# piotrmwojcik/GI-GS

Hardware: AMD Instinct MI355X
Metric: train-step renders/sec (fwd+bwd, G-buffer+indirect) at 800x800; PSNR vs the CPU oracle (higher is better)
Workload: dtype f32; 1 GPU; C2 (configs[1] TensoIR lego stand-in): 300k surface Gaussians, 800x800, SH deg 2, GI step=16 start=8 delta=0.0625; P=300000, N=640000, M=9, hip_graphs=on, fused_glue=on, gi_march=proj, rasterizer=whole step = 2 hand-captured hipGraphs (fwd, bwd), asynchronous binning

## Files before the change

gi-gs_amd/csrc/pbr.hip:

```cpp
#include <cmath>
#include <cstdlib>
#include <cstring>
#include <map>
#include <mutex>
#include <vector>

#include "gigs_common.h"
#include "pixel_ops.h"

namespace gigs {

__device__ __forceinline__ v3 safe_normalize(v3 v) {
  const float l = sqrtf(v.x * v.x + v.y * v.y + v.z * v.z);
  return l > 0.0f ? v3{v.x / l, v.y / l, v.z / l} : v3{0, 0, 0};
}
__device__ __forceinline__ v3 cube_dir_raw(float fx, float fy, int side) {
  switch (side) {
    case 0: return {1, -fy, -fx};
    case 1: return {-1, -fy, fx};
    case 2: return {fx, 1, fy};
    case 3: return {fx, -1, -fy};
    case 4: return {fx, -fy, 1};
    default: return {-fx, -fy, -1};
  }
}
__device__ __forceinline__ v3 cube_to_dir(int x, int y, int side, int N) {
  const float fx = 2.0f * (((float)x + 0.5f) / (float)N) - 1.0f;
  const float fy = 2.0f * (((float)y + 0.5f) / (float)N) - 1.0f;
  return safe_normalize(cube_dir_raw(fx, fy, side));
}
__device__ __forceinline__ float ndf_ggx(float alphaSqr, float cosTheta) {
  const float c = fminf(fmaxf(cosTheta, 0.0f), 1.0f);
  const float d = (c * alphaSqr - c) * c + 1.0f;
  return (float)((double)alphaSqr / ((double)(d * d) * 3.14159265358979323846));
}

__global__ void __launch_bounds__(256)
texel_table_kernel(int N, const float* __restrict__ area, float4* __restrict__ table) {
  const int o = blockIdx.x * 256 + threadIdx.x;
  if (o >= 6 * N * N) return;
  const int pz = o / (N * N), py = (o / N) % N, px = o % N;
  const v3 d = cube_to_dir(px, py, pz, N);
  float a = 1.0f;
  if (N > 1) {
    const int Hh = N / 2;
    a = area[abs(px - Hh)] * area[abs(py - Hh)];
  }
  table[o] = make_float4(d.x, d.y, d.z, a);
}

struct TexelTable { float4* dev = nullptr; };
static std::mutex g_table_mu;
static std::map<long long, TexelTable> g_table;

static const float4* texel_table(int N, hipStream_t s) {
  int dev = 0;
  if (hipGetDevice(&dev) != hipSuccess) return nullptr;
  std::lock_guard<std::mutex> lk(g_table_mu);
  const long long key = ((long long)dev << 32) | (unsigned)N;
  auto it = g_table.find(key);
  if (it != g_table.end()) return it->second.dev;
  const int Hh = N / 2;
  std::vector<float> h(Hh + 2, 1.0f);
  if (N > 1)
    for (int i = 0; i <= Hh; i++) h[i] = atanf((float)(i + 1) / (float)Hh) - atanf((float)i / (float)Hh);
  float* area = nullptr;
  TexelTable t;
  if (hipMalloc(&area, h.size() * sizeof(float)) != hipSuccess) return nullptr;
  if (hipMalloc(&t.dev, (size_t)6 * N * N * sizeof(float4)) != hipSuccess) return nullptr;
  if (hipMemcpyAsync(area, h.data(), h.size() * sizeof(float), hipMemcpyHostToDevice, s) != hipSuccess) return nullptr;
  hipLaunchKernelGGL(texel_table_kernel, dim3((6 * N * N + 255) / 256), dim3(256), 0, s, N, area, t.dev);
  if (hipStreamSynchronize(s) != hipSuccess) return nullptr;
  hipFree(area);
  g_table[key] = t;
  return t.dev;
}

template <int kCtrl, int kRowMask = 0xf>
__device__ __forceinline__ float pbr_dpp(float v) {
  return __int_as_float(__builtin_amdgcn_update_dpp(0, __float_as_int(v), kCtrl, kRowMask, 0xf, false));
}
__device__ __forceinline__ float wave_sum63(float v) {
  v += pbr_dpp<0xb1>(v);
  v += pbr_dpp<0x4e>(v);
  v += pbr_dpp<0x124>(v);
  v += pbr_dpp<0x128>(v);
  v += pbr_dpp<0x142, 0xa>(v);
  v += pbr_dpp<0x143, 0xc>(v);
  return v;
}

template <bool kBackward>
__global__ void __launch_bounds__(256)
diffuse_cubemap_kernel(int N, const float4* __restrict__ table, const float* __restrict__ src,
                       float* __restrict__ dst) {
  const int o = blockIdx.x * 4 + (threadIdx.x >> 6);
  const int lane = threadIdx.x & 63;
  if (o >= 6 * N * N) return;
  const float4 me = table[o];
  float c0 = 0, c1 = 0, c2 = 0;
  for (int i = lane; i < 6 * N * N; i += 64) {
    const float4 ot = table[i];
    const float d = kBackward ? (ot.x * me.x + ot.y * me.y + ot.z * me.z) : (me.x * ot.x + me.y * ot.y + me.z * ot.z);
    const float costheta = fminf(fmaxf(d, 0.0f), 0.999f);
    const float w = costheta * (kBackward ? me.w : ot.w) / 3.141592f;
    const float* t = src + 3 * (size_t)i;
    c0 += t[0] * w; c1 += t[1] * w; c2 += t[2] * w;
  }
  c0 = wave_sum63(c0); c1 = wave_sum63(c1); c2 = wave_sum63(c2);
  if (lane == 63) { dst[3 * (size_t)o] = c0; dst[3 * (size_t)o + 1] = c1; dst[3 * (size_t)o + 2] = c2; }
}


__global__ void __launch_bounds__(64)
specular_bounds_kernel(int N, float cutoff, float* __restrict__ bounds) {
  const int o = blockIdx.x * 64 + threadIdx.x;
  if (o >= 6 * N * N) return;
  const int pz = o / (N * N), py = (o / N) % N, px = o % N;
  const v3 VNR = cube_to_dir(px, py, pz, N);
  const int TILE = 16;
  for (int s = 0; s < 6; ++s) {
    int minx = N - 1, maxx = 0, miny = N - 1, maxy = 0;
    for (int tx = 0; tx < (N + TILE - 1) / TILE; tx++)
      for (int ty = 0; ty < (N + TILE - 1) / TILE; ty++) {
        const int tsx = tx * TILE, tsy = ty * TILE;
        const int tex = min((tx + 1) * TILE, N), tey = min((ty + 1) * TILE, N);
        const v3 L0 = cube_to_dir(tsx, tsy, s, N), L1 = cube_to_dir(tex, tsy, s, N);
        const v3 L2 = cube_to_dir(tsx, tey, s, N), L3 = cube_to_dir(tex, tey, s, N);
        const float mnx = fminf(fminf(L0.x, L1.x), fminf(L2.x, L3.x)), mxx = fmaxf(fmaxf(L0.x, L1.x), fmaxf(L2.x, L3.x));
        const float mny = fminf(fminf(L0.y, L1.y), fminf(L2.y, L3.y)), mxy = fmaxf(fmaxf(L0.y, L1.y), fmaxf(L2.y, L3.y));
        const float mnz = fminf(fminf(L0.z, L1.z), fminf(L2.z, L3.z)), mxz = fmaxf(fmaxf(L0.z, L1.z), fmaxf(L2.z, L3.z));
        const float maxdp = fmaxf(mnx * VNR.x, mxx * VNR.x) + fmaxf(mny * VNR.y, mxy * VNR.y) + fmaxf(mnz * VNR.z, mxz * VNR.z);
        if (maxdp >= cutoff) {
          for (int y = tsy; y < tey; ++y)
            for (int x = tsx; x < tex; ++x) {
              const v3 L = cube_to_dir(x, y, s, N);
              if (dot3(L, VNR) >= cutoff) {
                minx = min(minx, x); maxx = max(maxx, x);
                miny = min(miny, y); maxy = max(maxy, y);
              }
            }
        }
      }
    float* b = bounds + 24 * (size_t)o + s * 4;
    b[0] = (float)minx; b[1] = (float)maxx; b[2] = (float)miny; b[3] = (float)maxy;
  }
}

__device__ __forceinline__ v3 normalize_exact(v3 v) {
  const float l = sqrtf(v.x * v.x + v.y * v.y + v.z * v.z);
  if (!(l > 0x1p-60f && l < 0x1p60f)) return safe_normalize(v);
  const float r0 = __builtin_amdgcn_rcpf(l);
  const float e0 = __builtin_fmaf(-l, r0, 1.0f);
  const float r1 = __builtin_fmaf(e0, r0, r0);
  v3 q;
  {
    const float q0 = v.x * r1, e1 = __builtin_fmaf(-l, q0, v.x), q1 = __builtin_fmaf(e1, r1, q0);
    q.x = __builtin_fmaf(__builtin_fmaf(-l, q1, v.x), r1, q1);
  }
  {
    const float q0 = v.y * r1, e1 = __builtin_fmaf(-l, q0, v.y), q1 = __builtin_fmaf(e1, r1, q0);
    q.y = __builtin_fmaf(__builtin_fmaf(-l, q1, v.y), r1, q1);
  }
  {
    const float q0 = v.z * r1, e1 = __builtin_fmaf(-l, q0, v.z), q1 = __builtin_fmaf(e1, r1, q0);
    q.z = __builtin_fmaf(__builtin_fmaf(-l, q1, v.z), r1, q1);
  }
  return q;
}

template <bool kBackward>
__global__ void __launch_bounds__(256)
specular_cubemap_kernel(int N, const float4* __restrict__ table, const float* __restrict__ src,
                        const float* __restrict__ bounds, float roughness, float cutoff,
                        float* __restrict__ dst) {
  const int o = blockIdx.x * 4 + (threadIdx.x >> 6);
  const int lane = threadIdx.x & 63;
  if (o >= 6 * N * N) return;
  const int lx = lane & 7, ly = lane >> 3;
  const float4 me = table[o];
  const float alpha = roughness * roughness, alphaSqr = alpha * alpha;
  float wsum = 0.0f, c0 = 0, c1 = 0, c2 = 0;
  const int stride = kBackward ? 4 : 3;
  const float4* b4 = reinterpret_cast<const float4*>(bounds + 24 * (size_t)o);
  for (int s = 0; s < 6; ++s) {
    const float4 b = b4[s];
    const int xmin = (int)b.x, xmax = (int)b.y, ymin = (int)b.z, ymax = (int)b.w;
    if (xmin > xmax) continue;
    for (int y = ymin + ly; y <= ymax; y += 8)
      for (int x = xmin + lx; x <= xmax; x += 8) {
        const int i = (s * N + y) * N + x;
        const float4 ot = table[i];
        const float d = kBackward ? (me.x * ot.x + me.y * ot.y + me.z * ot.z) : (ot.x * me.x + ot.y * me.y + ot.z * me.z);
        if (d >= cutoff) {
          const float wiDotN = fmaxf(d, 0.0f);
          const v3 Hh = kBackward ? normalize_exact(v3{me.x + ot.x, me.y + ot.y, me.z + ot.z})
                                  : normalize_exact(v3{ot.x + me.x, ot.y + me.y, ot.z + me.z});
          const float VNRDotH = fmaxf(kBackward ? (ot.x * Hh.x + ot.y * Hh.y + ot.z * Hh.z)
                                                : (me.x * Hh.x + me.y * Hh.y + me.z * Hh.z), 0.0f);
          const float c = fminf(fmaxf(VNRDotH, 0.0f), 1.0f);
          const float dd = (c * alphaSqr - c) * c + 1.0f;
          const float ndf = alphaSqr / ((dd * dd) * 3.14159265358979323846f);
          const float w = wiDotN * ndf * (kBackward ? me.w : ot.w) / 4.0f;
          const float* t = src + (size_t)stride * i;
          c0 += t[0] * w; c1 += t[1] * w; c2 += t[2] * w;
          wsum += w;
        }
      }
  }
  c0 = wave_sum63(c0); c1 = wave_sum63(c1); c2 = wave_sum63(c2);
  if (!kBackward) wsum = wave_sum63(wsum);
  if (lane == 63) {
    if (kBackward) {
      float* q = dst + 3 * (size_t)o;
      q[0] = c0; q[1] = c1; q[2] = c2;
    } else {
      float* q = dst + 4 * (size_t)o;
      q[0] = c0; q[1] = c1; q[2] = c2; q[3] = wsum;
    }
  }
}


template <bool kSwap>
__global__ void __launch_bounds__(256)
specular_weights_kernel(int N, const float4* __restrict__ table, const float* __restrict__ bounds,
                        const uint32_t* __restrict__ offsets, float roughness, float cutoff,
                        float* __restrict__ W) {
  const int o = blockIdx.x * 4 + (threadIdx.x >> 6);
  const int lane = threadIdx.x & 63;
  if (o >= 6 * N * N) return;
  const float4 me = table[o];
  const float alpha = roughness * roughness, alphaSqr = alpha * alpha;
  const float4* b4 = reinterpret_cast<const float4*>(bounds + 24 * (size_t)o);
  for (int s = 0; s < 6; ++s) {
    const float4 b = b4[s];
    const int xmin = (int)b.x, xmax = (int)b.y, ymin = (int)b.z, ymax = (int)b.w;
    if (xmin > xmax || ymin > ymax) continue;
    const int wd = xmax - xmin + 1, n = wd * (ymax - ymin + 1);
    const float inv = 1.0f / (float)wd;
    const uint32_t base = offsets[6 * (size_t)o + s];
    for (int i = lane; i < n; i += 64) {
      const int yy = (int)(((float)i + 0.5f) * inv), xx = i - yy * wd;
      const float4 ot = table[(s * N + ymin + yy) * N + xmin + xx];
      const float d = kSwap ? (me.x * ot.x + me.y * ot.y + me.z * ot.z) : (ot.x * me.x + ot.y * me.y + ot.z * me.z);
      float f = -1.0f;
      if (d >= cutoff) {
        const float wiDotN = fmaxf(d, 0.0f);
        const v3 Hh = kSwap ? normalize_exact(v3{me.x + ot.x, me.y + ot.y, me.z + ot.z})
                            : normalize_exact(v3{ot.x + me.x, ot.y + me.y, ot.z + me.z});
        const float VNRDotH = fmaxf(kSwap ? (ot.x * Hh.x + ot.y * Hh.y + ot.z * Hh.z)
                                          : (me.x * Hh.x + me.y * Hh.y + me.z * Hh.z), 0.0f);
        const float c = fminf(fmaxf(VNRDotH, 0.0f), 1.0f);
        const float dd = (c * alphaSqr - c) * c + 1.0f;
        f = wiDotN * (alphaSqr / ((dd * dd) * 3.14159265358979323846f)) * (kSwap ? me.w : ot.w) / 4.0f;
      }
      W[(size_t)base + i] = f;
    }
  }
}

__global__ void __launch_bounds__(256)
specular_divide_weights_kernel(int N, const float* __restrict__ bounds, const uint32_t* __restrict__ offsets,
                               const float* __restrict__ W, const float* __restrict__ divisor, float* __restrict__ W2) {
  const int o = blockIdx.x * 4 + (threadIdx.x >> 6);
  const int lane = threadIdx.x & 63;
  if (o >= 6 * N * N) return;
  const float4* b4 = reinterpret_cast<const float4*>(bounds + 24 * (size_t)o);
  for (int s = 0; s < 6; ++s) {
    const float4 b = b4[s];
    const int xmin = (int)b.x, xmax = (int)b.y, ymin = (int)b.z, ymax = (int)b.w;
    if (xmin > xmax || ymin > ymax) continue;
    const int wd = xmax - xmin + 1, n = wd * (ymax - ymin + 1);
    const float inv = 1.0f / (float)wd;
    const uint32_t base = offsets[6 * (size_t)o + s];
    for (int i = lane; i < n; i += 64) {
      const int yy = (int)(((float)i + 0.5f) * inv), xx = i - yy * wd;
      const float w = W[(size_t)base + i];
      W2[(size_t)base + i] = w >= 0.0f ? w / divisor[(s * N + ymin + yy) * N + xmin + xx] : w;
    }
  }
}

template <int kLanes>
__device__ __forceinline__ float group_sum_last(float v) {
  v += pbr_dpp<0xb1>(v);
  v += pbr_dpp<0x4e>(v);
  if (kLanes == 8) return v + pbr_dpp<0x141>(v);
  v += pbr_dpp<0x124>(v);
  v += pbr_dpp<0x128>(v);
  if (kLanes == 64) {
    v += pbr_dpp<0x142, 0xa>(v);
    v += pbr_dpp<0x143, 0xc>(v);
  }
  return v;
}

template <bool kBackward, bool kNorm, int kLanes>
__device__ __forceinline__ void specular_apply_body(int block, int N, const float* __restrict__ src,
                                                    const float* __restrict__ bounds, const uint32_t* __restrict__ offsets,
                                                    const float* __restrict__ W, float* __restrict__ dst,
                                                    float* __restrict__ wsum_out) {
  constexpr int kPerWave = 64 / kLanes;
  constexpr int kU = 4;
  const int lane = threadIdx.x & 63;
  const int total = 6 * N * N;
  const int o_raw = (block * 4 + (threadIdx.x >> 6)) * kPerWave + lane / kLanes;
  const bool valid = o_raw < total;
  const int o = valid ? o_raw : total - 1;
  const int g = lane % kLanes;
  const int stride = (kBackward && !kNorm) ? 4 : 3;

  int wd[6], pre[7], base[6];
  float inv[6];
  const float4* b4 = reinterpret_cast<const float4*>(bounds + 24 * (size_t)o);
  const uint32_t first = offsets[6 * (size_t)o];
  pre[0] = 0;
#pragma unroll
  for (int s = 0; s < 6; ++s) {
    const float4 b = b4[s];
    const int xmin = (int)b.x, xmax = (int)b.y, ymin = (int)b.z, ymax = (int)b.w;
    const bool empty = xmin > xmax || ymin > ymax;
    wd[s] = empty ? 1 : xmax - xmin + 1;
    pre[s + 1] = pre[s] + (empty ? 0 : wd[s] * (ymax - ymin + 1));
    base[s] = empty ? 0 : (s * N + ymin) * N + xmin;
    inv[s] = __builtin_amdgcn_rcpf((float)wd[s]);
  }
  const int n = valid ? pre[6] : 0;
  const float* wrow = W + first;

  float wsum = 0.0f, c0 = 0, c1 = 0, c2 = 0;
  int f_wd, f_base, f_pre, f_end;
  float f_inv;
  auto find_face = [&](int i) {
    f_wd = wd[0]; f_base = base[0]; f_pre = 0; f_end = pre[1]; f_inv = inv[0];
#pragma unroll
    for (int k = 1; k < 6; k++) {
      const bool ge = i >= pre[k];
      f_wd = ge ? wd[k] : f_wd; f_base = ge ? base[k] : f_base; f_pre = ge ? pre[k] : f_pre;
      f_end = ge ? pre[k + 1] : f_end; f_inv = ge ? inv[k] : f_inv;
    }
  };
  find_face(g);
  for (int i0 = g; i0 < n; i0 += kLanes * kU) {
    float w[kU];
    int idx[kU];
    const bool cross = i0 + kLanes * (kU - 1) >= f_end && f_end < n;
    if (__any(cross)) {
#pragma unroll
      for (int u = 0; u < kU; u++) {
        const int i = i0 + kLanes * u;
        const bool in = i < n;
        const int ic = in ? i : 0;
        w[u] = in ? wrow[i] : -1.0f;
        find_face(ic);
        const int loc = ic - f_pre;
        const int yy = (int)(((float)loc + 0.5f) * f_inv), xx = loc - yy * f_wd;
        idx[u] = f_base + yy * N + xx;
      }
      find_face(min(i0 + kLanes * kU, n - 1));
    } else {
#pragma unroll
      for (int u = 0; u < kU; u++) {
        const int i = i0 + kLanes * u;
        const bool in = i < n;
        w[u] = in ? wrow[i] : -1.0f;
        const int loc = in ? i - f_pre : 0;
        const int yy = (int)(((float)loc + 0.5f) * f_inv), xx = loc - yy * f_wd;
        idx[u] = f_base + yy * N + xx;
      }
    }
    float t0[kU], t1[kU], t2[kU];
#pragma unroll
    for (int u = 0; u < kU; u++) {
      const float* t = src + (size_t)stride * idx[u];
      t0[u] = t[0]; t1[u] = t[1]; t2[u] = t[2];
    }
#pragma unroll
    for (int u = 0; u < kU; u++) {
      if (w[u] >= 0.0f) {
        c0 += t0[u] * w[u]; c1 += t1[u] * w[u]; c2 += t2[u] * w[u];
        wsum += w[u];
      }
    }
  }
  c0 = group_sum_last<kLanes>(c0); c1 = group_sum_last<kLanes>(c1); c2 = group_sum_last<kLanes>(c2);
  if (!kBackward) wsum = group_sum_last<kLanes>(wsum);
  if (g == kLanes - 1 && valid) {
    if (kBackward) {
      float* q = dst + 3 * (size_t)o;
      q[0] = c0; q[1] = c1; q[2] = c2;
    } else if (kNorm) {
      float* q = dst + 3 * (size_t)o;
      q[0] = c0 / wsum; q[1] = c1 / wsum; q[2] = c2 / wsum;
      wsum_out[o] = wsum;
    } else {
      float* q = dst + 4 * (size_t)o;
      q[0] = c0; q[1] = c1; q[2] = c2; q[3] = wsum;
    }
  }
}

template <bool kBackward, bool kNorm, int kLanes>
__global__ void __launch_bounds__(256)
specular_apply_kernel(int N, const float* __restrict__ src, const float* __restrict__ bounds,
                      const uint32_t* __restrict__ offsets, const float* __restrict__ W,
                      float* __restrict__ dst, float* __restrict__ wsum_out) {
  specular_apply_body<kBackward, kNorm, kLanes>(blockIdx.x, N, src, bounds, offsets, W, dst, wsum_out);
}

struct SpecLevel {
  int N, lanes, block_begin;
  const float* src;
  const float* bounds;
  const uint32_t* offsets;
  const float* W;
  float* dst;
  float* wsum_out;
};
struct SpecLevels { int n; SpecLevel lv[8]; };

template <bool kBackward>
__global__ void __launch_bounds__(256) specular_apply_multi_kernel(SpecLevels L) {
  int k = 0;
#pragma unroll
  for (int i = 1; i < 8; i++)
    if (i < L.n && (int)blockIdx.x >= L.lv[i].block_begin) k = i;
  const SpecLevel& v = L.lv[k];
  const int block = (int)blockIdx.x - v.block_begin;
  if (v.lanes == 8) specular_apply_body<kBackward, true, 8>(block, v.N, v.src, v.bounds, v.offsets, v.W, v.dst, v.wsum_out);
  else if (v.lanes == 16) specular_apply_body<kBackward, true, 16>(block, v.N, v.src, v.bounds, v.offsets, v.W, v.dst, v.wsum_out);
  else specular_apply_body<kBackward, true, 64>(block, v.N, v.src, v.bounds, v.offsets, v.W, v.dst, v.wsum_out);
}

static int spec_lanes_for(const Options& o, int avg_window) {
  return (avg_window > 0 && avg_window <= o.spec_max8) ? 8 : (avg_window > 0 && avg_window <= o.spec_max16) ? 16 : 64;
}

template <bool kBackward, bool kNorm>
static void launch_specular_apply(const Options& o, int res, int avg_window, const float* src, const float* bounds,
                                  const uint32_t* offsets, const float* W, float* dst, float* wsum_out, hipStream_t s) {
  const int total = 6 * res * res;
  const int max8 = o.spec_max8, max16 = o.spec_max16;
  if (avg_window > 0 && avg_window <= max8) {
    const int waves = (total + 7) / 8;
    hipLaunchKernelGGL((specular_apply_kernel<kBackward, kNorm, 8>), dim3((waves + 3) / 4), dim3(256), 0, s, res, src,
                       bounds, offsets, W, dst, wsum_out);
  } else if (avg_window > 0 && avg_window <= max16) {
    const int waves = (total + 3) / 4;
    hipLaunchKernelGGL((specular_apply_kernel<kBackward, kNorm, 16>), dim3((waves + 3) / 4), dim3(256), 0, s, res, src,
                       bounds, offsets, W, dst, wsum_out);
  } else {
    hipLaunchKernelGGL((specular_apply_kernel<kBackward, kNorm, 64>), dim3((total + 3) / 4), dim3(256), 0, s, res, src,
                       bounds, offsets, W, dst, wsum_out);
  }
}

__device__ __forceinline__ int cube_face_uv(float x, float y, float z, float& u, float& v) {
  const float ax = fabsf(x), ay = fabsf(y), az = fabsf(z);
  int idx;
  float c;
  if (az > fmaxf(ax, ay)) { idx = 4; c = z; }
  else if (ay > ax) { idx = 2; c = y; y = z; }
  else { idx = 0; c = x; x = z; }
  if (c < 0.f) idx += 1;
  const float m = (1.0f / fabsf(c)) * 0.5f;
  const float m0 = (idx == 0 || idx == 5) ? -m : m;
  const float m1 = (idx != 2) ? -m : m;
  u = x * m0 + 0.5f;
  v = y * m1 + 0.5f;
  if (!isfinite(u) || !isfinite(v)) return -1;
  u = fminf(fmaxf(u, 0.f), 1.f);
  v = fminf(fmaxf(v, 0.f), 1.f);
  return idx;
}

struct Taps { int idx[4]; float w[4]; };

__device__ __forceinline__ bool cube_taps(int res, float dx, float dy, float dz, Taps& t) {
  float u, v;
  const int face = cube_face_uv(dx, dy, dz, u, v);
  if (face < 0) return false;
  const float fu = u * (float)res - 0.5f, fv = v * (float)res - 0.5f;
  const float flu = floorf(fu), flv = floorf(fv);
  const int iu0 = (int)flu, iv0 = (int)flv;
  const float tu = fu - flu, tv = fv - flv;
  float wsum = 0.0f;
  bool dropped = false;
#pragma unroll
  for (int k = 0; k < 4; k++) {
    const int ox = k & 1, oy = k >> 1;
    const int ix = iu0 + ox, iy = iv0 + oy;
    const float w = (ox ? tu : 1.0f - tu) * (oy ? tv : 1.0f - tv);
    const bool out_x = ix < 0 || ix >= res, out_y = iy < 0 || iy >= res;
    int idx;
    if (!out_x && !out_y) {
      idx = (face * res + iy) * res + ix;
    } else if (out_x && out_y) {
      idx = -1;
      dropped = true;
    } else {
      const float a = 2.0f * (((float)ix + 0.5f) / (float)res) - 1.0f;
      const float b = 2.0f * (((float)iy + 0.5f) / (float)res) - 1.0f;
      const v3 d = cube_dir_raw(a, b, face);
      float u2, v2;
      const int f2 = cube_face_uv(d.x, d.y, d.z, u2, v2);
      const int x2 = min(res - 1, max(0, (int)floorf(u2 * (float)res)));
      const int y2 = min(res - 1, max(0, (int)floorf(v2 * (float)res)));
      idx = (f2 * res + y2) * res + x2;
    }
    t.idx[k] = idx;
    t.w[k] = w;
    if (idx >= 0) wsum += w;
  }
  if (dropped) {
#pragma unroll
    for (int k = 0; k < 4; k++) t.w[k] = t.idx[k] >= 0 ? t.w[k] / wsum : 0.0f;
  }
  return true;
}

__device__ __forceinline__ v3 cube_sample(const float* __restrict__ tex, const Taps& t) {
  v3 r = {0, 0, 0};
#pragma unroll
  for (int k = 0; k < 4; k++)
    if (t.idx[k] >= 0) {
      const float* p = tex + 3 * (size_t)t.idx[k];
      r.x += p[0] * t.w[k];
      r.y += p[1] * t.w[k];
      r.z += p[2] * t.w[k];
    }
  return r;
}

__global__ void __launch_bounds__(256)
cubemap_mip_fwd_kernel(int r, int C, const float* __restrict__ in, float* __restrict__ out) {
  const int i = blockIdx.x * 256 + threadIdx.x;
  if (i >= 6 * r * r * C) return;
  const int c = i % C, x = (i / C) % r, y = (i / (C * r)) % r, f = i / (C * r * r);
  const int R2 = 2 * r;
  const float* p = in + ((size_t)(f * R2 + 2 * y) * R2 + 2 * x) * C + c;
  out[i] = (p[0] + p[C] + p[(size_t)R2 * C] + p[(size_t)R2 * C + C]) * 0.25f;
}

__global__ void __launch_bounds__(256)
cubemap_mip_bwd_kernel(int r, const float* __restrict__ dout, float* __restrict__ din, const float* __restrict__ add,
                       const float* __restrict__ dout2) {
  const int res = 2 * r;
  const int i = blockIdx.x * 256 + threadIdx.x;
  if (i >= 6 * res * res) return;
  const int x = i % res, y = (i / res) % res, s = i / (res * res);
  const float start = -1.0f + 1.0f / (float)res, end = 1.0f - 1.0f / (float)res;
  const float stepv = (end - start) / (float)(res - 1);
  const float gx = x < res / 2 ? start + stepv * (float)x : end - stepv * (float)(res - 1 - x);
  const float gy = y < res / 2 ? start + stepv * (float)y : end - stepv * (float)(res - 1 - y);
  v3 d = cube_dir_raw(gx, gy, s);
  const float n = fmaxf(sqrtf(d.x * d.x + d.y * d.y + d.z * d.z), 1e-12f);
  d = {d.x / n, d.y / n, d.z / n};
  Taps t;
  v3 v = {0, 0, 0};
  if (cube_taps(r, d.x, d.y, d.z, t)) {
#pragma unroll
    for (int k = 0; k < 4; k++)
      if (t.idx[k] >= 0) {
        const float* p = dout + 3 * (size_t)t.idx[k];
        float p0 = p[0], p1 = p[1], p2 = p[2];
        if (dout2) {
          const float* q = dout2 + 3 * (size_t)t.idx[k];
          p0 += q[0]; p1 += q[1]; p2 += q[2];
        }
        v.x += (p0 * 0.25f) * t.w[k];
        v.y += (p1 * 0.25f) * t.w[k];
        v.z += (p2 * 0.25f) * t.w[k];
      }
  }
  if (add) {
    v.x += add[3 * (size_t)i]; v.y += add[3 * (size_t)i + 1]; v.z += add[3 * (size_t)i + 2];
  }
  din[3 * (size_t)i] = v.x; din[3 * (size_t)i + 1] = v.y; din[3 * (size_t)i + 2] = v.z;
}

__global__ void __launch_bounds__(256)
cube_texture_fwd_kernel(int res, const float* __restrict__ tex, int n, const float* __restrict__ dirs,
                        float* __restrict__ out, int planar) {
  const int i = blockIdx.x * 256 + threadIdx.x;
  if (i >= n) return;
  Taps t;
  v3 v = {0, 0, 0};
  if (cube_taps(res, dirs[3 * (size_t)i], dirs[3 * (size_t)i + 1], dirs[3 * (size_t)i + 2], t)) v = cube_sample(tex, t);
  if (planar) {
    out[i] = v.x; out[(size_t)n + i] = v.y; out[2 * (size_t)n + i] = v.z;
  } else {
    out[3 * (size_t)i] = v.x; out[3 * (size_t)i + 1] = v.y; out[3 * (size_t)i + 2] = v.z;
  }
}

__device__ __forceinline__ float torch_linspace(float start, float end, int n, int i) {
  if (n <= 1) return start;
  const float step = (end - start) / (float)(n - 1);
  return (i < n / 2) ? start + step * (float)i : end - step * (float)(n - 1 - i);
}
__global__ void __launch_bounds__(256)
latlong_to_cubemap_kernel(int res_y, int res_x, int Hl, int Wl, int C, const float* __restrict__ latlong,
                          float* __restrict__ cube) {
  const int i = blockIdx.x * 256 + threadIdx.x;
  const int n = 6 * res_y * res_x;
  if (i >= n) return;
  const int face = i / (res_y * res_x), rem = i - face * res_y * res_x;
  const int ty = rem / res_x, tx = rem - ty * res_x;
  const float gy = torch_linspace(-1.0f + 1.0f / (float)res_y, 1.0f - 1.0f / (float)res_y, res_y, ty);
  const float gx = torch_linspace(-1.0f + 1.0f / (float)res_x, 1.0f - 1.0f / (float)res_x, res_x, tx);
  float rx, ry, rz;
  switch (face) {
    case 0: rx = 1.0f; ry = -gy; rz = -gx; break;
    case 1: rx = -1.0f; ry = -gy; rz = gx; break;
    case 2: rx = gx; ry = 1.0f; rz = gy; break;
    case 3: rx = gx; ry = -1.0f; rz = -gy; break;
    case 4: rx = gx; ry = -gy; rz = 1.0f; break;
    default: rx = -gx; ry = -gy; rz = -1.0f; break;
  }
  const float inv = 1.0f / fmaxf(sqrtf(rx * rx + ry * ry + rz * rz), 1e-12f);
  rx *= inv; ry *= inv; rz *= inv;
  const float kPi = 3.14159265358979323846f;
  const float tu = atan2f(rx, -rz) / (2.0f * kPi) + 0.5f;
  const float tv = acosf(fminf(fmaxf(ry, -1.0f), 1.0f)) / kPi;
  const float u = tu * (float)Wl - 0.5f, v = tv * (float)Hl - 0.5f;
  const float fu0 = floorf(u), fv0 = floorf(v);
  const float fu = u - fu0, fv = v - fv0;
  auto wrap = [](int a, int m) { a %= m; return a < 0 ? a + m : a; };
  const int iu0 = wrap((int)fu0, Wl), iu1 = wrap((int)fu0 + 1, Wl);
  const int iv0 = wrap((int)fv0, Hl), iv1 = wrap((int)fv0 + 1, Hl);
  for (int c = 0; c < C; c++) {
    const float a = latlong[((size_t)iv0 * Wl + iu0) * C + c] * (1.0f - fu) + latlong[((size_t)iv0 * Wl + iu1) * C + c] * fu;
    const float b = latlong[((size_t)iv1 * Wl + iu0) * C + c] * (1.0f - fu) + latlong[((size_t)iv1 * Wl + iu1) * C + c] * fu;
    cube[(size_t)i * C + c] = a * (1.0f - fv) + b * fv;
  }
}

struct ShadeArgs {
  int H, W;
  const float *normals, *view_dirs, *albedo, *roughness;
  const uint8_t* mask;
  const float *occlusion, *metallic, *background;
  const float* diffuse; int diffuse_res;
  int L; const float* spec[8]; int spec_res[8];
  const float* lut; int lut_w, lut_h;
  int tone, gamma;
#ifdef GIGS_DIAG
  int ablate;
#endif
  int lds_total;
  int lds_diffuse_off;
  int lds_spec_off[8];
  float *render_rgb, *diffuse_rgb, *specular_rgb, *diffuse_light;
  const float *g_render, *g_diffuse_rgb, *g_specular_rgb, *g_diffuse_light;
  float *d_albedo, *d_roughness, *d_metallic, *d_diffuse;
  float* d_spec[8];
  int ps, cs;
  float rough_scale, rough_bias;
  float *out_F0, *out_linear, *out_roughness;
  const float *g_albedo_mul_a, *g_albedo_mul_b, *g_roughness_add, *g_metallic_add;
  const float *g_scale, *lamb_mask, *lamb_acc4;
};

__device__ __forceinline__ float get_mip(float r, int L, float& dmip_dr) {
  const float MINR = 0.08f, MAXR = 0.5f;
  if (r < MAXR) {
    const float c = fminf(fmaxf(r, MINR), MAXR);
    dmip_dr = (r >= MINR && r <= MAXR) ? (1.0f / (MAXR - MINR)) * (float)(L - 2) : 0.0f;
    return (c - MINR) / (MAXR - MINR) * (float)(L - 2);
  }
  const float c = fminf(fmaxf(r, MAXR), 1.0f);
  dmip_dr = (r >= MAXR && r <= 1.0f) ? 1.0f / (1.0f - MAXR) : 0.0f;
  return (c - MAXR) / (1.0f - MAXR) + (float)L - 2.0f;
}
__device__ __forceinline__ float aces(float x, float& d) {
  const float a = 2.51f, b = 0.03f, c = 2.43f, dd = 0.59f, e = 0.14f;
  const float num = x * (a * x + b), den = x * (c * x + dd) + e;
  d = ((2 * a * x + b) * den - num * (2 * c * x + dd)) / (den * den);
  return num / den;
}

struct ShadePix {
  v3 a, dl_raw, dl, drgb, sp, s0, s1, F0, refl, srgb;
  float r, occ, m, fgx, fgy, dfgx_dv, dfgy_dv, lf, dmdr;
  int l0, l1;
  bool lvl_inside;
  Taps td, t0, t1;
// ... 908 lines not shown
```

Measured before the change: 343.0 renders/s.

## Move per-face tables to LDS, prefetch weights, and pack specular accumulation

Moves the per-output six-face prefix, width and base tables from registers into a per-group shared-memory table, and face lookup becomes a count plus indexed LDS reads. Texel addressing is turned into byte offsets built with 24-bit multiplies and inline asm. Weights are software-prefetched one iteration ahead, and accumulation uses packed v_pk_add_f32 under an exec mask set with v_cmpx. The aim is lower register pressure and fewer address and compare instructions in the specular filter gather loop. In exchange it relies on fragile inline asm and wave-level fences, and adds LDS traffic on face crossings.

```diff
diff --git a/gi-gs_amd/csrc/pbr.hip b/gi-gs_amd/csrc/pbr.hip
--- a/gi-gs_amd/csrc/pbr.hip
+++ b/gi-gs_amd/csrc/pbr.hip
@@ -282,6 +282,8 @@
   }
 }
 
+typedef float pbr_f2 __attribute__((ext_vector_type(2)));
+
 template <int kLanes>
 __device__ __forceinline__ float group_sum_last(float v) {
   v += pbr_dpp<0xb1>(v);
@@ -311,79 +313,116 @@
   const int g = lane % kLanes;
   const int stride = (kBackward && !kNorm) ? 4 : 3;
 
-  int wd[6], pre[7], base[6];
-  float inv[6];
+  __shared__ int face_tab[4 * kPerWave * 20];
+  int* tab = face_tab + ((threadIdx.x >> 6) * kPerWave + lane / kLanes) * 20;
   const float4* b4 = reinterpret_cast<const float4*>(bounds + 24 * (size_t)o);
   const uint32_t first = offsets[6 * (size_t)o];
-  pre[0] = 0;
-#pragma unroll
-  for (int s = 0; s < 6; ++s) {
-    const float4 b = b4[s];
-    const int xmin = (int)b.x, xmax = (int)b.y, ymin = (int)b.z, ymax = (int)b.w;
-    const bool empty = xmin > xmax || ymin > ymax;
-    wd[s] = empty ? 1 : xmax - xmin + 1;
-    pre[s + 1] = pre[s] + (empty ? 0 : wd[s] * (ymax - ymin + 1));
-    base[s] = empty ? 0 : (s * N + ymin) * N + xmin;
-    inv[s] = __builtin_amdgcn_rcpf((float)wd[s]);
-  }
-  const int n = valid ? pre[6] : 0;
-  const float* wrow = W + first;
-
-  float wsum = 0.0f, c0 = 0, c1 = 0, c2 = 0;
-  int f_wd, f_base, f_pre, f_end;
+  int n_all;
+  {
+    int wd[6], pre[7], base[6];
+    pre[0] = 0;
+#pragma unroll
+    for (int s = 0; s < 6; ++s) {
+      const float4 b = b4[s];
+      const int xmin = (int)b.x, xmax = (int)b.y, ymin = (int)b.z, ymax = (int)b.w;
+      const bool empty = xmin > xmax || ymin > ymax;
+      wd[s] = empty ? 1 : xmax - xmin + 1;
+      pre[s + 1] = pre[s] + (empty ? 0 : wd[s] * (ymax - ymin + 1));
+      base[s] = empty ? 0 : (s * N + ymin) * N + xmin;
+    }
+    n_all = pre[6];
+    if (g == 0) {
+#pragma unroll
+      for (int s = 0; s < 7; ++s) tab[s] = pre[s];
+#pragma unroll
+      for (int s = 0; s < 6; ++s) { tab[8 + s] = wd[s]; tab[14 + s] = base[s]; }
+    }
+    __builtin_amdgcn_fence(__ATOMIC_RELEASE, "wavefront");
+    __builtin_amdgcn_wave_barrier();
+    __builtin_amdgcn_fence(__ATOMIC_ACQUIRE, "wavefront");
+  }
+  const int n = valid ? n_all : 0;
+  const uint32_t first0 = __builtin_amdgcn_readfirstlane(first);
+  const char* wbase = reinterpret_cast<const char*>(W + first0);
+  const char* tbase = reinterpret_cast<const char*>(src);
+  const int wrel = (int)(first - first0);
+  auto load_w = [&](int i) { return *reinterpret_cast<const float*>(wbase + (uint32_t)(4 * (wrel + i))); };
+
+  pbr_f2 acc01 = {0.0f, 0.0f}, accw2 = {0.0f, 0.0f};
+  int f_pre, f_end;
+  uint32_t f_off, f_row;
   float f_inv;
   auto find_face = [&](int i) {
-    f_wd = wd[0]; f_base = base[0]; f_pre = 0; f_end = pre[1]; f_inv = inv[0];
-#pragma unroll
-    for (int k = 1; k < 6; k++) {
-      const bool ge = i >= pre[k];
-      f_wd = ge ? wd[k] : f_wd; f_base = ge ? base[k] : f_base; f_pre = ge ? pre[k] : f_pre;
-      f_end = ge ? pre[k + 1] : f_end; f_inv = ge ? inv[k] : f_inv;
-    }
+    int k = 0;
+#pragma unroll
+    for (int j = 1; j < 6; j++) k += i >= tab[j] ? 1 : 0;
+    f_pre = tab[k]; f_end = tab[k + 1];
+    const int f_wd = tab[8 + k];
+    f_off = (uint32_t)(4 * stride * (tab[14 + k] - f_pre)); f_row = (uint32_t)(4 * stride * (N - f_wd));
+    f_inv = __builtin_amdgcn_rcpf((float)f_wd);
   };
+  auto texel_offset = [&](int i) {
+    const uint32_t row = (uint32_t)(int)(((float)(i - f_pre) + 0.5f) * f_inv), ui = (uint32_t)i;
+    uint32_t lin = (ui << (stride == 3 ? 2 : 4)) + f_off;
+    if (stride == 3) asm("v_lshl_add_u32 %0, %1, 3, %2" : "=v"(lin) : "v"(ui), "v"(lin));
+    return __umul24(row, f_row) + lin;
+  };
+  float wn[kU];
+  int ic[kU];
+#pragma unroll
+  for (int u = 0; u < kU; u++) { wn[u] = -1.0f; ic[u] = min(g + kLanes * u, n - 1); }
+  if (n > 0) {
+#pragma unroll
+    for (int u = 0; u < kU; u++) wn[u] = load_w(ic[u]);
+  }
   find_face(g);
   for (int i0 = g; i0 < n; i0 += kLanes * kU) {
     float w[kU];
-    int idx[kU];
+    uint32_t off[kU];
     const bool cross = i0 + kLanes * (kU - 1) >= f_end && f_end < n;
     if (__any(cross)) {
 #pragma unroll
       for (int u = 0; u < kU; u++) {
-        const int i = i0 + kLanes * u;
-        const bool in = i < n;
-        const int ic = in ? i : 0;
-        w[u] = in ? wrow[i] : -1.0f;
-        find_face(ic);
-        const int loc = ic - f_pre;
-        const int yy = (int)(((float)loc + 0.5f) * f_inv), xx = loc - yy * f_wd;
-        idx[u] = f_base + yy * N + xx;
+        find_face(ic[u]);
+        off[u] = texel_offset(ic[u]);
       }
       find_face(min(i0 + kLanes * kU, n - 1));
     } else {
 #pragma unroll
-      for (int u = 0; u < kU; u++) {
-        const int i = i0 + kLanes * u;
-        const bool in = i < n;
-        w[u] = in ? wrow[i] : -1.0f;
-        const int loc = in ? i - f_pre : 0;
-        const int yy = (int)(((float)loc + 0.5f) * f_inv), xx = loc - yy * f_wd;
-        idx[u] = f_base + yy * N + xx;
-      }
+      for (int u = 0; u < kU; u++) off[u] = texel_offset(ic[u]);
     }
     float t0[kU], t1[kU], t2[kU];
 #pragma unroll
     for (int u = 0; u < kU; u++) {
-      const float* t = src + (size_t)stride * idx[u];
+      const float* t = reinterpret_cast<const float*>(tbase + off[u]);
       t0[u] = t[0]; t1[u] = t[1]; t2[u] = t[2];
     }
 #pragma unroll
+    for (int u = 1; u < kU; u++) w[u] = i0 + kLanes * u < n ? wn[u] : -1.0f;
+    asm volatile("v_mov_b32 %0, %1" : "=v"(w[0]) : "v"(wn[0]));
+#pragma unroll
     for (int u = 0; u < kU; u++) {
-      if (w[u] >= 0.0f) {
-        c0 += t0[u] * w[u]; c1 += t1[u] * w[u]; c2 += t2[u] * w[u];
-        wsum += w[u];
-      }
-    }
-  }
+      ic[u] = min(i0 + kLanes * (kU + u), n - 1);
+      wn[u] = load_w(ic[u]);
+    }
+#pragma unroll
+    for (int u = 0; u < kU; u++) asm volatile("" : "+v"(t0[u]), "+v"(t1[u]), "+v"(t2[u]));
+#pragma unroll
+    for (int u = 0; u < kU; u++) {
+      const pbr_f2 wp = {w[u], t2[u] * w[u]};
+      const pbr_f2 p01 = {t0[u] * w[u], t1[u] * w[u]};
+      unsigned long long saved;
+      asm volatile("s_mov_b64 %[sv], exec\n\t"
+                   "v_cmpx_le_f32_e32 vcc, 0, %[w]\n\t"
+                   "v_pk_add_f32 %[a01], %[a01], %[p01]\n\t"
+                   "v_pk_add_f32 %[aw2], %[aw2], %[wp]\n\t"
+                   "s_mov_b64 exec, %[sv]"
+                   : [a01] "+v"(acc01), [aw2] "+v"(accw2), [sv] "=&s"(saved)
+                   : [w] "v"(w[u]), [p01] "v"(p01), [wp] "v"(wp)
+                   : "vcc");
+    }
+  }
+  float c0 = acc01.x, c1 = acc01.y, c2 = accw2.y, wsum = accw2.x;
   c0 = group_sum_last<kLanes>(c0); c1 = group_sum_last<kLanes>(c1); c2 = group_sum_last<kLanes>(c2);
   if (!kBackward) wsum = group_sum_last<kLanes>(wsum);
   if (g == kLanes - 1 && valid) {
```

After: 348.4 renders/s, median of 6. 1.6% higher.
